# 1dayac/spades_for_blackbird

Hardware: AMD Instinct MI355X
Metric: distinct k-mers/sec (k=21, 150 bp synthetic reads, count only) (higher is better)
Workload: dtype u64

## Files before the change

### spades_for_blackbird_amd/csrc/msd.hip

```cpp
#include <hip/hip_runtime.h>

#include <algorithm>
#include <chrono>
#include <cmath>
#include <cstdio>
#include <cstdlib>
#include <cstring>
#include <optional>
#include <type_traits>
#include <vector>

#include "bbk_internal.h"
#include "kmer_ops.h"
#include "msd.h"

namespace bbk {

#ifndef BBK_KEYS_TILE
#define BBK_KEYS_TILE 8192
#endif
#ifndef BBK_KEYS_THREADS
#define BBK_KEYS_THREADS 512
#endif
template <int W>
// ... 2620 lines not shown
    uint32_t vals[kItems] = {};
    part_tail<1, kItems, kThreads, MAXB, false, false>(keys, vals, binrank, lhist, lstart, goff, scan_tmp, stage,
                                                       vals_unused, nb, T.gbin0, L, cursor, out, nullptr, 0, 0ull);
}

static size_t part_view_smem() {
    return part_smem(1, PartCfg<1>::TILE, false, false, true) + (size_t)kViewSpan * (4 + 2);
}

__global__ void k_view_recanon(const uint64_t *__restrict__ in, const uint32_t *__restrict__ seg_off,
                               const uint32_t *__restrict__ seg_size, int k, uint64_t *__restrict__ out, uint64_t cap,
                               uint32_t *__restrict__ count) {
    const uint32_t o = seg_off[blockIdx.x], n = seg_size[blockIdx.x];
    const uint64_t mask = (1ull << (2 * k)) - 1ull;
    const int lane = threadIdx.x & 63;
    for (uint32_t i0 = 0; i0 < n; i0 += blockDim.x) {
        const uint32_t i = i0 + threadIdx.x;
        Key<1> x;
        x.w[0] = 0;
        bool keep = false;
        if (i < n) {
            x.w[0] = in[o + i] & mask;
            keep = !kmer_less_nucl<1>(kmer_rc<1>(x, k), x);
        }
        const uint64_t bal = __ballot(keep);
        uint32_t base = 0;
        if (lane == 0 && bal) base = atomicAdd(count, (uint32_t)__popcll(bal));
        base = __shfl(base, 0);
        const uint64_t at = (uint64_t)base + __popcll(bal & ((1ull << lane) - 1ull));
        if (keep && at < cap) out[at] = x.w[0];
    }
}

void BucketView::materialise(bbk_ctx *ctx) {
    if (!live()) return;
    keys.alloc(n() * 8 + 16);
    if (nbuckets) {
        KernelTimer t(ctx, "compact", (double)D * (4 + 8));
        hipLaunchKernelGGL(k_compact_narrow<false>, dim3((unsigned)(((uint64_t)nbuckets * 64 + 255) / 256)), dim3(256), 0,
                           ctx->stream, slots.as<uint32_t>(), nullptr, dcount.as<uint32_t>(), off.as<uint64_t>(), nbuckets,
                           stride, seg.as<uint16_t>(), hb, keys.as<uint64_t>(), nullptr);
        check_launch("compact");
    }
    if (n_extra)
        BBK_HIP(bbk::copy_async(keys.as<uint64_t>() + D, extra.p, n_extra * 8, hipMemcpyDeviceToDevice, ctx->stream));
    stream_wait(ctx);
    release_slots();
}

template <int W>
struct BktCfg {
#ifndef BBK_BKT_NT
#define BBK_BKT_NT 512
#define BBK_BKT_ITEMS 11
#endif
#ifndef BBK_BKT2_NT
#define BBK_BKT2_NT 512
#define BBK_BKT2_ITEMS 7
#endif
    static constexpr int NT = (W == 1) ? BBK_BKT_NT : BBK_BKT2_NT;
    static constexpr int ITEMS = (W == 1) ? BBK_BKT_ITEMS : (W == 2 ? BBK_BKT2_ITEMS : (W == 3 ? 5 : 3));
    static constexpr uint32_t CAP = NT * ITEMS;
    static constexpr int NT2 = 512;
    static constexpr int ITEMS2 = (W == 1) ? 23 : (W == 2 ? 11 : (W == 3 ? 7 : 5));
    static constexpr uint32_t CAP2 = NT2 * ITEMS2;
};
constexpr double kBucketFill = 0.70;

static double wall() { return std::chrono::duration<double>(std::chrono::steady_clock::now().time_since_epoch()).count(); }

struct MsdKnobs {
    struct PerProcess {
        bool no_dist = getenv("BBK_NO_DIST") != nullptr;
        uint32_t hash_max_probes = (uint32_t)env_u64(getenv("BBK_HASH_MAX_PROBES"), kHashMaxProbes);
        uint64_t pass_limit = env_u64(getenv("BBK_PASS_LIMIT"), 0);
        bool no_narrow = getenv("BBK_NO_NARROW") != nullptr;
        bool xcd_slots = env_u64(getenv("BBK_XCD_SLOTS"), 1) != 0;
        bool xcd_tiles = env_u64(getenv("BBK_XCD_TILES"), 1) != 0;
        bool no_narrow_b = getenv("BBK_NO_NARROW_B") != nullptr;
        bool no_bucket_handoff = getenv("BBK_NO_BUCKET_HANDOFF") != nullptr;
        uint32_t nw_wgs_per_cu = (uint32_t)env_u64(getenv("BBK_NW_WGS_PER_CU"), 0);
    };
    const PerProcess &once = *[] {
        static const PerProcess p;
        return &p;
    }();
    bool no_slots = getenv("BBK_NO_SLOTS") != nullptr;
    bool no_kslots = getenv("BBK_NO_KSLOTS") != nullptr;
    uint64_t slots_min = env_u64(getenv("BBK_SLOTS_MIN"), 1ull << 22);
    bool verbose = getenv("BBK_VERBOSE") != nullptr;
    bool no_direct = getenv("BBK_NO_DIRECT") != nullptr;
    bool no_level0 = getenv("BBK_NO_LEVEL0") != nullptr;
    bool no_part_kslots = getenv("BBK_NO_PART_KSLOTS") != nullptr;
};

enum class Outcome {
    Declined,
    Done,
    TooBig,
    SlotsGaveUp,
    KeySlotsGaveUp,
    NeedDense,
};

struct MsdInput {
    const bbk_reads *rd;
    const void *keys;
    const uint32_t *vals;
    uint64_t n;
    bool with_mask;
    BucketView *view = nullptr;
};
// ... 96 lines not shown
    }

    double plan_fill(bool from_reads) const { return (!from_reads && use_hash_dedup()) ? 0.52 : kBucketFill; }
    uint64_t pass_limit(bool from_reads) const {
        if (knobs.once.pass_limit) return knobs.once.pass_limit;
        return (uint64_t)(plan_fill(from_reads) * 512 * 0.75 * kMaxBins * bucket_cap() * 0.98);
    }

    struct Sel {
        uint32_t lo = 0, span = 0;
        int shl = 0;
        uint32_t mul = 0;
        uint64_t est = 0;
        void finish() {
            shl = __builtin_clz(span - 1u);
            const uint64_t S = (uint64_t)span << shl;
            mul = S >= (1ull << 32) ? 0u : (uint32_t)((((1ull << 32) - S) << 32) / S);
        }
    };
    struct Dst {
        void *keys = nullptr;
        uint32_t *vals = nullptr;
    };

    struct Plan {
        uint64_t N;
        uint64_t Ntot;
        double target;
        uint32_t nb1 = 1;
        int b1 = 0;
        bool too_deep;
        int nw_hb;
        bool narrow, hslots, kslots, slots;
        uint32_t rd_tile, ntiles1, ntiles1h;
        int xs;
        uint32_t nsub, sub_cap, seg_cap, cap2, stride2, spill_cap;
        size_t rec_ab;
    };

    Plan plan(uint64_t N, uint64_t n_chunks, bool from_reads, bool has_val, const Sel &sel, bool has_dst) const {
        Plan P;
        const bool ranged = sel.span != 0;
        P.Ntot = N;
        P.N = N = ranged ? sel.est : N;
        BBK_REQUIRE(N < (1ull << 32) - kPartTileK, BBK_ERR_ARG,
                    "batch holds %llu records%s; one pass is limited to 2^32-1 (split the input)",
                    (unsigned long long)N, ranged ? " in one range of the prefix space" : "");

        const double fill = plan_fill(from_reads);
        P.target = fill * bucket_cap();
        const double want = std::max(1.0, std::ceil((double)N / P.target));
        while (P.nb1 < 512 && (double)P.nb1 * P.nb1 < want) {
            P.nb1 <<= 1;
            ++P.b1;
        }
        const int ref_bits = dmode == MSD_REF ? std::max(0, 4 - (ranged ? sel.shl : 0)) : 0;
        if (P.b1 < ref_bits) {
            P.b1 = ref_bits;
            P.nb1 = 1u << P.b1;
        }
        const bool u32_slots = (double)N / fill * 1.1 + (double)N < 4.2e9;
        P.nw_hb = (int)(2 * k) - 32;
        P.narrow = W == 1 && from_reads && !ranged && !has_dst && P.nw_hb >= 1 && P.nw_hb <= 10 && slots_ok &&
                   dmode == MSD_HASH && use_hash_dedup() && N >= knobs.slots_min && !knobs.once.no_narrow && u32_slots &&
                   (double)N / kNwBins1 / P.target < 0.75 * kMaxBins;
        if (P.narrow) {
            P.b1 = 10;
            P.nb1 = kNwBins1;
        }
        P.too_deep = want / P.nb1 > 0.75 * kMaxBins;
        if (P.too_deep) return P;

        P.rd_tile = P.narrow ? (uint32_t)(has_val ? NwCfg<true>::CHUNKS : NwCfg<false>::CHUNKS) : (uint32_t)kRdThreads;
        P.ntiles1 = from_reads ? (uint32_t)((n_chunks + P.rd_tile - 1) / P.rd_tile)
                               : (uint32_t)((P.Ntot + kPartTileK - 1) / kPartTileK);
        P.ntiles1h = (uint32_t)((n_chunks + kRdHistThreads - 1) / kRdHistThreads);

        P.hslots = slots_ok && !has_dst && dmode == MSD_HASH && (use_hash_dedup() || use_hashidx_dedup()) && P.nb1 > 1 &&
                   N >= knobs.slots_min && u32_slots;
        P.kslots = kslots_ok && slots_ok && (even_part || (!has_dst && !ranged && expand_k != 0)) && !from_reads &&
                   assume_distinct && (dmode == MSD_KEYS || dmode == MSD_REF) && P.nb1 > 1 && N >= knobs.slots_min &&
                   !knobs.no_direct && u32_slots;
        P.slots = P.hslots || P.kslots;
        BBK_REQUIRE(!P.narrow || P.slots, BBK_ERR_INTERNAL, "narrow records need the slot mode");
        P.xs = (P.slots && knobs.once.xcd_slots && ctx->num_xcds == 8) ? 3 : 0;
        P.nsub = P.nb1 << P.xs;
        P.sub_cap = P.xs ? ((uint32_t)((double)N / P.nsub * 1.06) + 2048u) | 1u : 0u;
        P.seg_cap = !P.slots ? 0u
                    : P.xs   ? P.sub_cap << P.xs
                             : ((uint32_t)((double)N / P.nb1 * (P.kslots ? 1.06 : 1.01)) + 8192u) | 1u;
        P.cap2 = P.narrow ? (uint32_t)(kNwHashThreads * kNwHashItems) : bucket_cap();
        P.rec_ab = P.narrow ? 4 : rec;
        P.stride2 = P.cap2 + (uint32_t)(256 / P.rec_ab);
        P.spill_cap = P.slots ? (uint32_t)(N / 8 + 65536) : 0u;
        return P;
    }

    struct Pass {
        static constexpr uint32_t kFlagCap = 65536;
        MsdRunner &R;
        bbk_ctx *ctx;
        const MsdInput &in;
        MsdOutput &out;
        const Sel sel;
        const Dst dst;
        const bool from_reads, has_val, ranged, has_dst, out_vals, need_vbuf, verbose;
        Plan P{};
        uint64_t N = 0, n_chunks = 0;
        DevBuf coff, tile_read, tiles_h;
        enum { kCtlSpill = 0, kCtlUnordered = 4, kCtlDup = 8, kCtlFlagN = 12, kCtlDbg = 16, kCtlTotal = 32, kCtlWords = 40 };
        DevBuf ctl;
        uint32_t h_ctl[kCtlWords] = {};
        uint32_t *ctl_at(int w) const { return ctl.as<uint32_t>() + w; }
        uint64_t *ctl_total() const { return reinterpret_cast<uint64_t *>(ctl_at(kCtlTotal)); }
        uint64_t h_total() const {
            uint64_t t;
            memcpy(&t, h_ctl + kCtlTotal, 8);
            return t;
        }
        ReadSrc S{}, Sh{};
        TileMap M1{}, M2{};
        PartLevel L1{}, L2{};
        DevBuf spill_k, spill_v;
        DevBuf hist1, cur1, bufA, valA;
        uint32_t n32 = 0;
        std::vector<uint32_t> h1, off1, tstart, snb2, sbin, hsub, fill1;
        std::vector<uint32_t> over_seg;
        uint32_t nbuckets = 0, ntiles2 = 0, nwg2 = 0;
        bool narrow_b = false;
        uint32_t *stage = nullptr;
        DevBuf layout_d;
        uint32_t *seg_tile = nullptr, *seg_off = nullptr, *seg_nb2 = nullptr, *seg_bin = nullptr, *seg_size = nullptr,
                 *xstart_d = nullptr;
        DevBuf desc2, desc2h, hist2, boff, bufB, valB;
        std::vector<uint32_t> xstart;
        DevBuf dcount, slot_off, bseg, bbase, flag_ids;
        DevBuf c64, d64;
        bool d64_scanned = false;
        std::vector<DevBuf> scan_keep;
        BucketArgs A{};
        bool direct = false;
        uint32_t ctr[4] = {0, 0, 0, 0};
        std::vector<uint32_t> flagged, hd, hb;
        std::vector<uint32_t> big;
        uint32_t hbo[2] = {0, 0};
        MsdOutput extra;
        uint64_t novf = 0;

        Pass(MsdRunner &r, const MsdInput &i, MsdOutput &o, const Sel &s, Dst d)
            : R(r), ctx(r.ctx), in(i), out(o), sel(s), dst(d), from_reads(i.rd != nullptr),
              has_val(i.with_mask || i.vals != nullptr), ranged(s.span != 0), has_dst(d.keys != nullptr),
              out_vals(r.op != MSD_OP_NONE), need_vbuf(has_val || out_vals), verbose(r.knobs.verbose) {}

        double rec_bytes(uint64_t n) const { return (double)n * (rec + (has_val ? 4 : 0)); }
        uint32_t *vals_or_null(DevBuf &b) const { return has_val ? b.as<uint32_t>() : nullptr; }

        Outcome run(uint64_t *n_records = nullptr) {
            ctl.alloc(kCtlWords * 4);
            BBK_HIP(hipMemsetAsync(ctl.p, 0, kCtlWords * 4, ctx->stream));
            count_instances();
            out.instances = N;
            out.n = 0;
            if (N == 0) return empty();
            if (!ranged && n_records && N > R.pass_limit(from_reads)) {
                *n_records = N;
                return Outcome::TooBig;
            }
            P = R.plan(N, n_chunks, from_reads, has_val, sel, has_dst);
            N = P.N;
            if (in.view && !view_level1()) return Outcome::NeedDense;
            if (P.too_deep) {
                if (verbose) fprintf(stderr, "[bbk] msd declines: N=%llu needs more than two levels\n", (unsigned long long)N);
                return Outcome::Declined;
            }
            level1_tiles();
            if (auto r = level1()) return *r;
            level2_layout();
            level2_scatter();
            if (auto r = first_pass()) return *r;
            if (auto r = overflow()) return *r;
            compact();
            return Outcome::Done;
        }

        bool view_level1() const {
            return W == 1 && !P.too_deep && P.kslots && R.expand_k && !ranged && !has_dst && !R.even_part && !has_val;
        }

        Outcome empty() {
            if (!has_dst) {
                out.keys.alloc(16);
                out.vals.alloc(16);
            }
            return Outcome::Done;
        }

        void count_instances() {
            N = (R.expand_k && !from_reads) ? 2 * in.n : in.n;
            if (!from_reads) return;
            const bbk_reads *rd = in.rd;
            BBK_REQUIRE(R.dmode == MSD_HASH, BBK_ERR_INTERNAL, "reads are partitioned by hash prefix only");
// ... 103 lines not shown
            if (P.narrow) {
                if constexpr (W == 1) {
                    const double pbn = (double)in.rd->n_words * 8 + (double)N * (4 + (has_val ? 4 : 0));
                    const uint32_t per_cu = R.knobs.once.nw_wgs_per_cu;
                    const uint32_t grid = per_cu ? std::min<uint32_t>(P.ntiles1, (uint32_t)ctx->num_cus * per_cu) : P.ntiles1;
                    R.launch(has_val ? k_part_reads_narrow<true> : k_part_reads_narrow<false>, "k_part_reads_narrow", pbn,
                             grid, kNwThreads, part_reads_narrow_smem(has_val), S, L1, P.ntiles1, S.tiles,
                             cur1.as<uint32_t>(), bufA.as<uint32_t>(), vals_or_null(valA));
                }
            } else {
                const double pb = (from_reads ? (double)in.rd->n_words * 8 : rec_bytes(N)) + rec_bytes(N);
                if (from_reads)
                    R.template launch_part_reads<false>("k_part_reads", pb, P.ntiles1, has_val, S, L1, nullptr,
                                                        cur1.as<uint32_t>(), bufA.as<Key<W>>(), valA.as<uint32_t>());
                else if (in.view)
                    level1_from_view();
                else
                    R.template scatter_keys<true>(has_val, "k_part_l1", pb, P.ntiles1, (const Key<W> *)in.keys, in.vals, M1, L1,
                                   cur1.as<uint32_t>(), bufA.as<Key<W>>(), valA.as<uint32_t>());
            }
            if (!P.slots) return std::nullopt;
            auto r = slot_fills();
            if (in.view && !r) {
                in.view->release_slots();
                if (verbose) fprintf(stderr, "[bbk] msd key slots: level 1 read stage A's buckets (%llu + %llu keys)\n",
                                     (unsigned long long)in.view->D, (unsigned long long)in.view->n_extra);
            }
            return r;
        }

        void level1_from_view() {
            if constexpr (W == 1) {
                BucketView &v = *in.view;
                const uint32_t half = kPartTileK / 2;
                const uint32_t nt = (uint32_t)((v.D + half - 1) / half);
                if (nt) {
                    DevBuf vdesc((size_t)nt * sizeof(uint2) + 16);
                    hipLaunchKernelGGL(k_view_tile_desc, dim3((nt + 255) / 256), dim3(256), 0, ctx->stream,
                                       v.off.as<uint64_t>(), v.nbuckets, v.D, half, nt, vdesc.as<uint2>());
                    check_launch("k_view_tile_desc");
                    TileMap Mv = M1;
                    Mv.n = 2 * v.D;
                    Mv.ntiles = nt;
                    R.launch(R.expand_tag ? k_part_view<true> : k_part_view<false>, "k_part_view",
                             (double)v.D * 4 + 2.0 * (double)v.D * rec, nt, PartCfg<1>::THREADS, part_view_smem(),
                             v.slots.as<uint32_t>(), v.off.as<uint64_t>(), v.seg.as<uint16_t>(), vdesc.as<uint2>(),
                             v.stride, v.hb, Mv, L1, cur1.as<uint32_t>(), bufA.as<Key<1>>());
                }
                if (v.n_extra) {
                    TileMap Me = M1;
                    Me.n = 2 * v.n_extra;
                    const uint32_t nte = (uint32_t)((Me.n + kPartTileK - 1) / kPartTileK);
                    R.template scatter_keys<true>(false, "k_part_l1", rec_bytes(v.n_extra) + rec_bytes(Me.n), nte,
                                                  v.extra.as<Key<W>>(), nullptr, Me, L1, cur1.as<uint32_t>(),
                                                  bufA.as<Key<W>>(), nullptr);
                }
            }
        }

        Outcome give_up_key_slots() {
            if constexpr (W == 1) {
                if (in.view && !in.view->live() && !in.view->keys.p) {
                    BucketView &v = *in.view;
                    const uint64_t n = v.n();
                    v.keys.alloc(n * rec + 16);
                    DevBuf cnt(16);
                    BBK_HIP(hipMemsetAsync(cnt.p, 0, 16, ctx->stream));
                    hipLaunchKernelGGL(k_view_recanon, dim3(P.nsub), dim3(256), 0, ctx->stream, bufA.as<uint64_t>(),
                                       seg_off, seg_size, (int)R.expand_k,
                                       v.keys.as<uint64_t>(), n, cnt.as<uint32_t>());
                    check_launch("k_view_recanon");
                    uint32_t got = 0;
                    BBK_HIP(hipMemcpyAsync(&got, cnt.p, 4, hipMemcpyDeviceToHost, ctx->stream));
                    stream_wait(ctx);
                    BBK_REQUIRE(got == n, BBK_ERR_INTERNAL, "canonical keys rebuilt from level 1: %u of %llu", got,
                                (unsigned long long)n);
                }
            }
            return Outcome::KeySlotsGaveUp;
        }

        std::optional<Outcome> slot_fills() {
            const uint32_t nsub = P.nsub, xs = P.xs;
            std::vector<uint32_t> c1(nsub);
            BBK_HIP(hipMemcpyAsync(c1.data(), cur1.p, (size_t)nsub * 4, hipMemcpyDeviceToHost, ctx->stream));
            stream_wait(ctx);
            uint64_t got = 0;
            const uint32_t cap1 = xs ? P.sub_cap : P.seg_cap;
            for (uint32_t b = 0; b < P.nb1; ++b) {
                bool over = false;
                uint32_t tot = 0;
                for (uint32_t s2 = b << xs; s2 < (b + 1) << xs; ++s2) {
                    const uint32_t reserved = c1[s2] - off1[s2];
                    got += reserved;
                    over = over || reserved > cap1;
                    fill1[s2] = std::min(reserved, cap1);
                    tot += fill1[s2];
                }
                if (over) over_seg.push_back(b);
                h1[b] = over ? 0u : tot;
                for (uint32_t s2 = b << xs; s2 < (b + 1) << xs; ++s2) hsub[s2] = over ? 0u : fill1[s2];
            }
            if (got > P.Ntot) {
// ... 13 lines not shown
                            (unsigned long long)got, (unsigned long long)P.Ntot);
            }
            if (ranged) {
                N = got;
                out.instances = N;
            }
            BBK_REQUIRE(got == N, BBK_ERR_INTERNAL, "level-1 reservations do not add up (%llu vs %llu)",
                        (unsigned long long)got, (unsigned long long)N);
            if (N == 0) return empty();
            if (P.kslots && !over_seg.empty()) {
                if (verbose) fprintf(stderr, "[bbk] msd key slots: %zu segments overflow, exact mode\n", over_seg.size());
                return Outcome::KeySlotsGaveUp;
            }
            return std::nullopt;
        }

        static size_t pad4(size_t words) { return (words + 7) & ~(size_t)3; }
        size_t layout_words(uint32_t *off_w) const {
            const size_t len[6] = {(size_t)P.nsub + 1, (size_t)P.nsub + 1, P.nb1, (size_t)P.nb1 + 1, P.nsub, P.nsub};
            size_t at = 0;
            for (int i = 0; i < 6; ++i) {
                if (off_w) off_w[i] = (uint32_t)at;
                at += pad4(len[i]);
            }
            return at;
        }

        void level2_layout() {
            const uint32_t nb1 = P.nb1, nsub = P.nsub, xs = P.xs;
            if (!P.slots)
                for (uint32_t b = 0; b < nb1; ++b) hsub[b] = h1[b];
            tstart[0] = 0;
            sbin[0] = 0;
            const uint32_t tile2 = P.narrow ? (uint32_t)(has_val ? Nw2Cfg<true>::TILE : Nw2Cfg<false>::TILE) : kPartTileK;
            for (uint32_t s2 = 0; s2 < nsub; ++s2) tstart[s2 + 1] = tstart[s2] + (hsub[s2] + tile2 - 1) / tile2;
            for (uint32_t b = 0; b < nb1; ++b) {
                snb2[b] = (uint32_t)std::min<double>(kMaxBins, std::max(1.0, std::ceil((double)h1[b] / P.target)));
                sbin[b + 1] = sbin[b] + snb2[b];
            }
            nbuckets = sbin[nb1];

            const int w0bits = R.w0bits();
            uint64_t span_b = 0;
            for (uint32_t b = 0; b < nb1; ++b)
                if (h1[b]) {
                    const uint64_t Q = 1ull << (32 - P.b1), q = (Q + snb2[b] - 1) / snb2[b];
                    span_b = std::max(span_b, w0bits > 32 ? q << (w0bits - 32) : q >> (32 - w0bits));
                }
            narrow_b = W == 1 && P.kslots && !R.even_part && !ranged && !has_dst && !has_val && R.op == MSD_OP_NONE &&
                       R.dmode == MSD_KEYS && span_b <= (1ull << 32) && !R.knobs.once.no_narrow_b;
            if (P.kslots && verbose)
                fprintf(stderr, "[bbk] msd key slots: %s records from level 2 (widest bucket 2^%.1f keys)\n",
                        narrow_b ? "4-byte" : "8-byte", std::log2((double)std::max<uint64_t>(span_b, 1)));

            ntiles2 = tstart[nsub];
            nwg2 = ntiles2;
            if (R.knobs.once.xcd_tiles && ntiles2) {
                xstart.resize(nsub);
                uint32_t per_xcd[8] = {0, 0, 0, 0, 0, 0, 0, 0};
                for (uint32_t s2 = 0; s2 < nsub; ++s2) {
                    uint32_t &c = per_xcd[(s2 >> xs) & 7u];
                    xstart[s2] = c;
                    c += tstart[s2 + 1] - tstart[s2];
                }
                nwg2 = 8u * *std::max_element(per_xcd, per_xcd + 8);
            }
            uint32_t off_w[6];
            const size_t words = layout_words(off_w);
            layout_d.alloc(words * 4);
            uint32_t *h = stage + pad4(nsub), *d = layout_d.as<uint32_t>();
            memcpy(h + off_w[0], tstart.data(), ((size_t)nsub + 1) * 4);
            memcpy(h + off_w[1], off1.data(), ((size_t)nsub + 1) * 4);
            memcpy(h + off_w[2], snb2.data(), (size_t)nb1 * 4);
            memcpy(h + off_w[3], sbin.data(), ((size_t)nb1 + 1) * 4);
            memcpy(h + off_w[4], hsub.data(), (size_t)nsub * 4);
            if (!xstart.empty()) memcpy(h + off_w[5], xstart.data(), (size_t)nsub * 4);
            BBK_HIP(hipMemcpyAsync(d, h, words * 4, hipMemcpyHostToDevice, ctx->stream));
            seg_tile = d + off_w[0];
            seg_off = d + off_w[1];
            seg_nb2 = d + off_w[2];
            seg_bin = d + off_w[3];
            seg_size = d + off_w[4];
            xstart_d = xstart.empty() ? nullptr : d + off_w[5];
            L2 = PartLevel{2, P.b1, nb1, R.dmode, w0bits, seg_nb2, seg_bin, sel.lo, sel.span, sel.shl, sel.mul};
            M2 = TileMap{seg_tile, seg_off, seg_size, nsub, N, ntiles2, 1, nullptr, 0, 0};
            desc2.alloc((size_t)nwg2 * sizeof(uint4) + 16);
            if (ntiles2) {
                if (xstart_d) BBK_HIP(hipMemsetAsync(desc2.p, 0, (size_t)nwg2 * sizeof(uint4), ctx->stream));
                hipLaunchKernelGGL(P.narrow ? k_tile_desc_narrow : k_tile_desc, dim3((ntiles2 + 255) / 256), dim3(256), 0,
                                   ctx->stream, M2, seg_nb2, seg_bin, tile2, xs, (const uint32_t *)xstart_d,
                                   desc2.as<uint4>());
                check_launch("k_tile_desc");
            }
            M2.desc = desc2.as<uint4>();
            if (!P.slots && xstart_d && !P.narrow) {
                desc2h.alloc((size_t)ntiles2 * sizeof(uint4) + 16);
                hipLaunchKernelGGL(k_tile_desc, dim3((ntiles2 + 255) / 256), dim3(256), 0, ctx->stream, M2, seg_nb2, seg_bin,
                                   kPartTileK, xs, (const uint32_t *)nullptr, desc2h.as<uint4>());
                check_launch("k_tile_desc");
            }
        }

        void level2_scatter() {
            hist2.alloc((size_t)nbuckets * 4 + 16);
            boff.alloc(((size_t)nbuckets + 1) * 4 + 16);
            const uint64_t nB = P.slots ? (uint64_t)nbuckets * P.stride2 : N;
            if (P.slots) BBK_REQUIRE(nB + N < (1ull << 32), BBK_ERR_INTERNAL, "slot layout exceeds 32-bit offsets");
            bufB.alloc(nB * (narrow_b ? 4 : P.rec_ab));
            if (need_vbuf) valB.alloc(nB * 4);
            if (!P.slots) {
                BBK_HIP(hipMemsetAsync(hist2.p, 0, (size_t)nbuckets * 4 + 16, ctx->stream));
                TileMap M2h = M2;
                if (desc2h.p) M2h.desc = desc2h.as<uint4>();
                R.template launch_part<false, true, false>("k_part_hist2", (double)N * rec, ntiles2, bufA.as<Key<W>>(), nullptr,
                                                    M2h, L2, hist2.as<uint32_t>(), nullptr, nullptr, nullptr);
                DevBuf h64(((size_t)nbuckets + 1) * 8);
                hipLaunchKernelGGL(k_u32_to_u64, dim3((nbuckets + 255) / 256), dim3(256), 0, ctx->stream,
                                   hist2.as<uint32_t>(), (uint64_t)nbuckets, h64.as<uint64_t>(), 0u);
                check_launch("k_u32_to_u64");
                const uint64_t tot = exclusive_scan_u64(ctx, h64.as<uint64_t>(), h64.as<uint64_t>(), nbuckets);
                BBK_REQUIRE(tot == N, BBK_ERR_INTERNAL, "level-2 histogram does not add up");
                hipLaunchKernelGGL(k_scan_to_u32, dim3((nbuckets + 1 + 255) / 256), dim3(256), 0, ctx->stream,
                                   h64.as<uint64_t>(), (uint64_t)nbuckets, tot, (const uint64_t *)nullptr,
                                   boff.as<uint32_t>());
                check_launch("k_scan_to_u32");
                BBK_HIP(bbk::copy_async(hist2.p, boff.p, (size_t)nbuckets * 4, hipMemcpyDeviceToDevice, ctx->stream));
                stream_wait(ctx);
            } else {
                if (P.narrow) bseg.alloc(((size_t)nbuckets + 1) * 2);
                hipLaunchKernelGGL(k_bucket_init, dim3((nbuckets + 255) / 256), dim3(256), 0, ctx->stream,
                                   hist2.as<uint32_t>(), nbuckets, P.stride2, (const uint32_t *)seg_bin, P.nb1,
                                   P.narrow ? bseg.as<uint16_t>() : (uint16_t *)nullptr);
                check_launch("k_bucket_init");
                use_slots(L2, P.cap2, P.stride2);
            }
            if (P.narrow) {
                if (ntiles2)
                    R.launch(has_val ? k_part_narrow2<true> : k_part_narrow2<false>, "k_part_narrow2",
                             2.0 * (double)N * (4 + (has_val ? 4 : 0)), nwg2, kNw2Threads, part_narrow2_smem(has_val),
                             bufA.as<uint32_t>(), vals_or_null(valA), desc2.as<uint4>(), L2, hist2.as<uint32_t>(),
                             bufB.as<uint32_t>(), vals_or_null(valB));
            } else if (narrow_b) {
                if constexpr (W == 1)
                    R.template launch_part<false, false, false, true>("k_part_l2", (double)N * (rec + 4), nwg2,
                                                                        bufA.as<Key<W>>(), nullptr, M2, L2, nullptr,
                                                                        hist2.as<uint32_t>(), bufB.as<Key<W>>(), nullptr);
            } else {
                R.template scatter_keys<false>(has_val, "k_part_l2", 2.0 * rec_bytes(N), nwg2, bufA.as<Key<W>>(), valA.as<uint32_t>(), M2,
                               L2, hist2.as<uint32_t>(), bufB.as<Key<W>>(), valB.as<uint32_t>());
            }
        }

        std::optional<Outcome> first_pass() {
            dcount.alloc((size_t)nbuckets * 4 + 16);
            A = BucketArgs{boff.as<uint32_t>(), dcount.as<uint32_t>(), nullptr, (int)R.k,
                           verbose ? ctl_at(kCtlDbg) : nullptr, P.slots ? P.cap2 : 0u, P.slots ? P.stride2 : 0u,
                           hist2.as<uint32_t>(), nullptr, nullptr, nullptr, ~0ull, R.knobs.once.hash_max_probes, nullptr};
            direct = (!P.slots || P.kslots) && R.assume_distinct && (R.dmode == MSD_KEYS || R.dmode == MSD_REF) &&
                     !R.knobs.no_direct;
            if (P.kslots) {
                c64.alloc(((size_t)nbuckets + 1) * 8);
                const ScanSrc src{hist2.p, SCAN_SLOT_FILL, P.stride2, P.cap2};
                uint64_t *const so = c64.as<uint64_t>();
                exclusive_scan_enqueue(ctx, 1, &src, &so, nbuckets, ctl_total(), false, scan_keep);
                slot_off.alloc(((size_t)nbuckets + 1) * 4 + 16);
                hipLaunchKernelGGL(k_scan_to_u32, dim3((nbuckets + 1 + 255) / 256), dim3(256), 0, ctx->stream,
                                   c64.as<uint64_t>(), (uint64_t)nbuckets, 0ull, (const uint64_t *)ctl_total(),
                                   slot_off.as<uint32_t>());
                check_launch("k_scan_to_u32");
                A.out_off = slot_off.as<uint32_t>();
            }
            if (direct) {
                if (!has_dst) {
                    out.keys.alloc(N * rec + 16);
                    if (out_vals) out.vals.alloc(N * 4 + 16);
                }
                A.sorted_keys = has_dst ? dst.keys : out.keys.p;
                A.sorted_vals = has_dst ? dst.vals : out.vals.as<uint32_t>();
                A.dup_flag = ctl_at(kCtlDup);
                A.strip_mask = R.strip_mask;
            }
            launch_buckets();
            flag_ids.alloc((size_t)kFlagCap * 4);
            if (P.hslots && !direct) {
                d64.alloc(((size_t)nbuckets + 1) * 8);
                const ScanSrc src{dcount.p, SCAN_U32_FLAGGED, 0u, 0u};
                uint64_t *const so = d64.as<uint64_t>();
                exclusive_scan_enqueue(ctx, 1, &src, &so, nbuckets, ctl_total(), false, scan_keep);
                d64_scanned = true;
            }
            fetch_flags();
            if (P.kslots && h_total() != N) {
                if (verbose) fprintf(stderr, "[bbk] msd key slots: %llu of %llu records placed, exact mode\n",
                                     (unsigned long long)h_total(), (unsigned long long)N);
                out.keys.release();
                out.vals.release();
                return give_up_key_slots();
            }
            if (!direct) return std::nullopt;
            if (ctr[2] == 0 && ctr[3] == 0 && (!P.kslots || ctr[0] == 0)) {
                out.n = N;
                out.nbuckets = 0;
// ... 8 lines not shown
                                     ctr[2], ctr[3]);
                out.keys.release();
                out.vals.release();
                return give_up_key_slots();
            }
            if (verbose) fprintf(stderr, "[bbk] msd direct output withdrawn (flagged=%u dup=%u): in-place pass\n", ctr[2], ctr[3]);
            if (!has_dst) {
                out.keys.release();
                out.vals.release();
            }
            A.sorted_keys = nullptr;
            A.sorted_vals = nullptr;
            A.dup_flag = nullptr;
            A.strip_mask = ~0ull;
            R.template bucket_dispatch<false>(nbuckets, bufB.as<Key<W>>(), valB.as<uint32_t>(), A, rec_bytes(N));
            fetch_flags();
            return std::nullopt;
        }

        void launch_buckets() {
            if (P.narrow) {
                if constexpr (W == 1) {
                    if (nbuckets)
                        with_op(R.op, [&](auto o) {
                            constexpr int OP = decltype(o)::value;
                            R.launch(k_bucket_hash32<OP>, "k_bucket_hash32", (double)N * (4 + (has_val ? 4 : 0)), nbuckets,
                                     kNwHashThreads, bucket_hash32_smem<OP>(), bufB.as<uint32_t>(), valB.as<uint32_t>(), A,
                                     bseg.as<uint16_t>(), P.nw_hb);
                        });
                }
            } else if (narrow_b) {
                if constexpr (W == 1) {
                    BBK_REQUIRE(direct, BBK_ERR_INTERNAL, "4-byte stage-B records need the direct output");
                    bbase.alloc(((size_t)nbuckets + 1) * 8);
                    if (nbuckets) {
                        hipLaunchKernelGGL(k_bucket_base, dim3((nbuckets + 255) / 256), dim3(256), 0, ctx->stream,
                                           (const uint32_t *)seg_nb2, (const uint32_t *)seg_bin, P.nb1, nbuckets, P.b1,
                                           R.w0bits(), bbase.as<uint64_t>());
                        check_launch("k_bucket_base");
                        constexpr int NT = BktCfg<1>::NT, IT = BktCfg<1>::ITEMS;
                        R.launch(k_bucket_dist_nb<NT, IT>, "k_bucket_dist", (double)N * (4 + rec), nbuckets, NT,
                                 bucket_dist_nb_smem<NT, IT>(), bufB.as<uint32_t>(), bbase.as<uint64_t>(), A);
                    }
                }
            } else {
                R.template bucket_dispatch<false>(nbuckets, bufB.as<Key<W>>(), valB.as<uint32_t>(), A, rec_bytes(N));
            }
        }

        void fetch_flags() {
            uint32_t *d_flag_n = P.slots ? ctl_at(kCtlSpill) + 2 : ctl_at(kCtlFlagN);
            if (!P.slots) BBK_HIP(hipMemsetAsync(d_flag_n, 0, 16, ctx->stream));
            hipLaunchKernelGGL(k_flagged, dim3((nbuckets + 255) / 256), dim3(256), 0, ctx->stream, dcount.as<uint32_t>(),
                               nbuckets, flag_ids.as<uint32_t>(), kFlagCap, d_flag_n);
            check_launch("k_flagged");
            BBK_HIP(hipMemcpyAsync(h_ctl, ctl.p, kCtlWords * 4, hipMemcpyDeviceToHost, ctx->stream));
            stream_wait(ctx);
            if (P.slots) memcpy(ctr, h_ctl + kCtlSpill, 12);
            else ctr[2] = h_ctl[kCtlFlagN];
            if (direct) ctr[3] = h_ctl[kCtlDup];
        }

        std::optional<Outcome> overflow() {
            const uint32_t n_flag = ctr[2];
            if (n_flag > kFlagCap) {
                if (verbose) fprintf(stderr, "[bbk] msd: %u buckets overflow\n", n_flag);
                return P.slots ? Outcome::SlotsGaveUp : Outcome::Declined;
            }
            flagged.resize(n_flag);
            if (n_flag) {
                BBK_HIP(hipMemcpyAsync(flagged.data(), flag_ids.p, (size_t)n_flag * 4, hipMemcpyDeviceToHost, ctx->stream));
                stream_wait(ctx);
// ... 642 lines not shown
```

Baseline: 27.90 billion.

## Use 4-byte records from level 1 with hash tag applied at level 2

Adds a 'late tag' path for key-slot partitioning from a view. Level 1 now emits 4-byte low-bit records binned by the top 10 bits of both orientations, and the hash tag is computed only at level 2. Level 2 then folds the tag into its bin index, and new permutation kernels reorder the slot-fill scan to match. The goal is to halve record traffic in the first partition pass. The cost is a more complex bucket mapping, extra small kernels, and a forced 1024-bin level 1.

```diff
diff --git a/spades_for_blackbird_amd/csrc/msd.hip b/spades_for_blackbird_amd/csrc/msd.hip
--- a/spades_for_blackbird_amd/csrc/msd.hip
+++ b/spades_for_blackbird_amd/csrc/msd.hip
@@ -2676,6 +2676,321 @@
     }
 }
 
+constexpr int kLtThreads = 1024;
+constexpr int kLt1Items = 14;
+constexpr int kLt2Items = 12;
+
+struct LtLds {
+    uint32_t *lhist;
+    uint2 *tab;
+    uint32_t *lstart, *scan_tmp;
+    unsigned long long *mark;
+    uint16_t *mbase, *nz;
+    uint32_t *stage;
+};
+template <int ITEMS>
+__device__ __forceinline__ LtLds lt_lds(unsigned char *smem) {
+    constexpr int MW = kLtThreads * ITEMS / 64;
+    LtLds S;
+    S.lhist = reinterpret_cast<uint32_t *>(smem);
+    S.tab = reinterpret_cast<uint2 *>(smem);
+    S.lstart = S.lhist + 2 * kMaxBins;
+    S.scan_tmp = S.lstart + kMaxBins;
+    S.mark = reinterpret_cast<unsigned long long *>(S.scan_tmp + 64);
+    S.mbase = reinterpret_cast<uint16_t *>(S.mark + MW);
+    S.nz = S.mbase + MW;
+    S.stage = reinterpret_cast<uint32_t *>(S.nz + kMaxBins);
+    return S;
+}
+static size_t lt_smem(int items, size_t more) {
+    const size_t tile = (size_t)kLtThreads * items;
+    return sizeof(uint32_t) * (3 * kMaxBins + 64) + (tile / 64) * (8 + 2) + (size_t)kMaxBins * 2 + tile * 4 + more;
+}
+
+__device__ inline uint64_t lt_tagged(uint32_t seg, uint32_t lo, int lobits, int k) {
+    Key<1> x;
+    x.w[0] = ((uint64_t)seg << lobits) | lo;
+    return x.w[0] | (__umul64hi(xxh3_64<1>(x), 16ull) << (2 * k));
+}
+
+template <int ITEMS, class KeyOf>
+__device__ __forceinline__ void lt_tail(const LtLds &S, const uint32_t (&lo)[ITEMS], const uint32_t (&bins)[ITEMS / 2],
+                                        uint32_t nb, uint32_t *__restrict__ cur, uint64_t slot_end, uint32_t rec_or,
+                                        const PartLevel &L, uint32_t *__restrict__ out, KeyOf key_of) {
+    constexpr int NT = kLtThreads, MW = NT * ITEMS / 64;
+    static_assert(ITEMS % 2 == 0 && ITEMS <= 32 && NT * ITEMS < 65536, "packed bins, one bit per item, 16-bit positions");
+    const uint32_t tid = threadIdx.x;
+    const int lane = tid & 63, wave = tid >> 6;
+    const uint32_t c = tid < nb ? S.lhist[tid] : 0u;
+    uint32_t incl = c;
+    incl = wave_scan_incl(incl);
+    const unsigned long long nzb = __ballot(c != 0);
+    if (lane == 63) S.scan_tmp[wave] = incl | ((uint32_t)__popcll(nzb) << 16);
+    __syncthreads();
+    uint32_t before, total;
+    wave_totals<NT / 64>(S.scan_tmp, lane, wave, before, total);
+    const uint32_t staged = total & 0xFFFFu;
+    const uint32_t ex = (before & 0xFFFFu) + incl - c;
+    const uint32_t myr = (before >> 16) + (uint32_t)__popcll(nzb & ((1ull << lane) - 1ull));
+    S.lstart[tid] = ex;
+    uint32_t greserve = 0;
+    if (c) {
+        greserve = atomicAdd(cur, c);
+        S.nz[myr] = (uint16_t)tid;
+        atomicOr(&S.mark[ex >> 6], 1ull << (ex & 63u));
+    }
+    __syncthreads();
+#pragma unroll
+    for (int i = 0; i < ITEMS; ++i) {
+        const uint32_t bin = (bins[i >> 1] >> (16 * (i & 1))) & 0xFFFFu;
+        if (bin != 0xFFFFu) {
+            const uint32_t pos = atomicAdd(&S.lstart[bin], 1u);
+            S.stage[pos] = lo[i];
+        }
+    }
+    asm volatile("" : "+v"(greserve));
+    if (c) {
+        const int64_t room = (int64_t)slot_end - (int64_t)greserve;
+        S.tab[myr] = make_uint2(greserve - ex, (uint32_t)(int32_t)(room < -(int64_t)0x7FFF0000 ? -(int64_t)0x7FFF0000 : room) + ex);
+    }
+    if (wave == 0) {
+        constexpr int WPL = (MW + 63) / 64;
+        uint32_t pw[WPL], tot = 0;
+#pragma unroll
+        for (int j = 0; j < WPL; ++j) {
+            const int idx = lane * WPL + j;
+            pw[j] = tot;
+            tot += idx < MW ? (uint32_t)__popcll(S.mark[idx]) : 0u;
+        }
+        uint32_t inc2 = tot;
+        inc2 = wave_scan_incl(inc2);
+        const uint32_t lb = inc2 - tot;
+#pragma unroll
+        for (int j = 0; j < WPL; ++j) {
+            const int idx = lane * WPL + j;
+            if (idx < MW) S.mbase[idx] = (uint16_t)(lb + pw[j]);
+        }
+    }
+    __syncthreads();
+    const unsigned long long upto = (2ull << lane) - 1ull;
+    const unsigned long long *wmark = S.mark + wave;
+    const uint16_t *wmbase = S.mbase + wave;
+    uint32_t full = 0;
+#pragma unroll
+    for (int i = 0; i < ITEMS; ++i) {
+        const uint32_t pos = (uint32_t)i * NT + tid;
+        if (pos < staged) {
+            const uint32_t r = (uint32_t)wmbase[i * (NT / 64)] + (uint32_t)__popcll(wmark[i * (NT / 64)] & upto) - 1u;
+            unsigned long long e = reinterpret_cast<const unsigned long long *>(S.tab)[r];
+            const uint32_t rec = S.stage[pos];
+            asm volatile("" : "+v"(e));
+            if ((int32_t)pos >= (int32_t)(uint32_t)(e >> 32)) full |= 1u << i;
+            else out[(uint32_t)e + pos] = rec | rec_or;
+        }
+    }
+    if (full) {
+#pragma unroll 1
+        for (int i = 0; i < ITEMS; ++i) {
+            if ((full >> i) & 1u) {
+                const uint32_t pos = (uint32_t)i * NT + tid;
+                const uint32_t r = (uint32_t)wmbase[i * (NT / 64)] + (uint32_t)__popcll(wmark[i * (NT / 64)] & upto) - 1u;
+                const uint32_t sp = atomicAdd(L.spill_count, 1u);
+                if (sp < L.spill_cap) reinterpret_cast<uint64_t *>(L.spill_keys)[sp] = key_of((uint32_t)S.nz[r], S.stage[pos]);
+            }
+        }
+    }
+}
+
+template <bool DENSE>
+__global__ __launch_bounds__(kLtThreads) __attribute__((amdgpu_waves_per_eu(8, 8))) void k_part_view_lt(
+    const uint32_t *__restrict__ slots, const uint64_t *__restrict__ off, const uint16_t *__restrict__ seg,
+    const uint2 *__restrict__ vdesc, uint32_t stride, int hb, const uint64_t *__restrict__ dense, uint64_t nkeys_all, int k,
+    PartLevel L, uint32_t *__restrict__ cursor, uint32_t *__restrict__ out) {
+    constexpr int NT = kLtThreads, ITEMS = kLt1Items, KPT = NT * ITEMS / 2, MW = NT * ITEMS / 64;
+    extern __shared__ __attribute__((aligned(16))) unsigned char smem[];
+    const LtLds S = lt_lds<ITEMS>(smem);
+    uint32_t *toff = S.stage + NT * ITEMS;
+    uint16_t *tseg = reinterpret_cast<uint16_t *>(toff + kViewSpan);
+    const uint32_t tid = threadIdx.x;
+    uint32_t xcc = 0;
+    if (L.xcd_shift) {
+        asm volatile("s_getreg_b32 %0, hwreg(HW_REG_XCC_ID)" : "=s"(xcc));
+        xcc &= (1u << L.xcd_shift) - 1u;
+    }
+    const int lobits = 2 * k - 10;
+    const uint32_t lomask = lobits >= 32 ? 0xFFFFFFFFu : (1u << lobits) - 1u;
+    const uint64_t c0 = (uint64_t)blockIdx.x * KPT;
+    const uint64_t left = nkeys_all - c0;
+    const uint32_t nkeys = left < (uint64_t)KPT ? (uint32_t)left : (uint32_t)KPT;
+    uint32_t b0 = 0, span = 0;
+    bool staged_tab = false;
+    if (!DENSE) {
+        const uint2 d = vdesc[blockIdx.x];
+        b0 = d.x;
+        span = d.y - d.x + 1u;
+        staged_tab = span <= (uint32_t)kViewSpan;
+        if (staged_tab && tid < span) {
+            toff[tid] = (uint32_t)off[b0 + tid];
+            tseg[tid] = seg[b0 + tid];
+        }
+    }
+    S.lhist[tid] = 0;
+    if (tid < 2 * MW) reinterpret_cast<uint32_t *>(S.mark)[tid] = 0u;
+    __syncthreads();
+
+    uint64_t x[ITEMS / 2];
+    if (DENSE) {
+#pragma unroll
+        for (int j = 0; j < ITEMS / 2; ++j) {
+            const uint32_t cl = (uint32_t)(j * NT) + tid;
+            x[j] = dense[c0 + (cl < nkeys ? cl : nkeys - 1u)];
+        }
+    } else {
+        uint32_t w[ITEMS / 2], sg[ITEMS / 2];
+#pragma unroll
+        for (int j = 0; j < ITEMS / 2; ++j) {
+            const uint32_t cl = (uint32_t)(j * NT) + tid;
+            const uint32_t c = (uint32_t)c0 + (cl < nkeys ? cl : nkeys - 1u);
+            uint32_t b, base;
+            if (staged_tab) {
+                uint32_t i = 0, hi = span;
+                while (hi - i > 1) {
+                    const uint32_t mid = (i + hi) >> 1;
+                    if (toff[mid] <= c) i = mid;
+                    else hi = mid;
+                }
+                b = b0 + i;
+                base = toff[i];
+                sg[j] = tseg[i];
+            } else {
+                b = view_bucket(off, b0, b0 + span, c);
+                base = (uint32_t)off[b];
+                sg[j] = seg[b];
+            }
+            w[j] = slots[(size_t)b * stride + (c - base)];
+        }
+#pragma unroll
+        for (int j = 0; j < ITEMS / 2; ++j) x[j] = nw_key(sg[j], w[j], hb);
+    }
+    uint32_t lo[ITEMS], bins[ITEMS / 2];
+#pragma unroll
+    for (int j = 0; j < ITEMS / 2; ++j) {
+        Key<1> a;
+        a.w[0] = x[j];
+        const uint64_t r = kmer_rc<1>(a, k).w[0];
+        const uint32_t ba = (uint32_t)(x[j] >> lobits), br = (uint32_t)(r >> lobits);
+        lo[2 * j] = (uint32_t)x[j] & lomask;
+        lo[2 * j + 1] = (uint32_t)r & lomask;
+        bins[j] = 0xFFFFFFFFu;
+        if ((uint32_t)(j * NT) + tid < nkeys) {
+            bins[j] = ba | (br << 16);
+            atomicAdd(&S.lhist[ba], 1u);
+            atomicAdd(&S.lhist[br], 1u);
+        }
+    }
+    __syncthreads();
+    const uint64_t slot_end = (uint64_t)tid * L.slot_stride + (L.xcd_shift ? (uint64_t)(xcc + 1u) * L.sub_cap : (uint64_t)L.slot_cap);
+    lt_tail<ITEMS>(S, lo, bins, (uint32_t)kMaxBins, &cursor[(tid << L.xcd_shift) + xcc], slot_end, 0u, L, out,
+                   [&](uint32_t bin, uint32_t rec) { return lt_tagged(bin, rec, lobits, k); });
+}
+
+__global__ __launch_bounds__(kLtThreads) __attribute__((amdgpu_waves_per_eu(8, 8))) void k_part_lt2(
+    const uint32_t *__restrict__ in, const uint4 *__restrict__ desc, int k, PartLevel L, uint32_t *__restrict__ cursor,
+    uint32_t *__restrict__ out) {
+    constexpr int NT = kLtThreads, ITEMS = kLt2Items, MW = NT * ITEMS / 64;
+    extern __shared__ __attribute__((aligned(16))) unsigned char smem[];
+    const LtLds S = lt_lds<ITEMS>(smem);
+    const uint32_t tid = threadIdx.x;
+    const uint4 d = desc[blockIdx.x];
+    const uint32_t begin = d.x, count = d.y, nb = d.z & 0xFFFFu, sgm = d.z >> 16, gbin0 = d.w;
+    if (count == 0) return;
+    const int lobits = 2 * k - 10;
+    const uint32_t nsub = nb >> 4;
+    const uint64_t segbits = (uint64_t)sgm << lobits;
+    S.lhist[tid] = 0;
+    if (tid < 2 * MW) reinterpret_cast<uint32_t *>(S.mark)[tid] = 0u;
+    __syncthreads();
+    uint32_t lo[ITEMS], bins[ITEMS / 2];
+#pragma unroll
+    for (int i = 0; i < ITEMS; ++i) {
+        const uint32_t local = (uint32_t)i * NT + tid;
+        lo[i] = in[begin + (local < count ? local : count - 1u)];
+    }
+#pragma unroll
+    for (int i = 0; i < ITEMS; ++i) asm volatile("" : "+v"(lo[i]));
+#pragma unroll
+    for (int i = 0; i < ITEMS; ++i) {
+        Key<1> x;
+        x.w[0] = segbits | lo[i];
+        const uint32_t tag = (uint32_t)__umul64hi(xxh3_64<1>(x), 16ull);
+        const uint32_t b = tag * nsub + __umulhi(lo[i] << (32 - lobits), nsub);
+        const bool valid = (uint32_t)i * NT + tid < count;
+        if (valid) atomicAdd(&S.lhist[b], 1u);
+        const uint32_t b16 = valid ? b : 0xFFFFu;
+        if (i & 1) bins[i >> 1] |= b16 << 16;
+        else bins[i >> 1] = b16;
+    }
+    __syncthreads();
+    const uint64_t slot_end = (uint64_t)(gbin0 + tid) * L.slot_stride + L.slot_cap;
+    lt_tail<ITEMS>(S, lo, bins, nb, &cursor[gbin0 + tid], slot_end, (uint32_t)segbits, L, out,
+                   [&](uint32_t, uint32_t rec) { return lt_tagged(sgm, rec, lobits, k); });
+}
+
+__global__ void k_bucket_base_lt(const uint32_t *__restrict__ seg_nb2, const uint32_t *__restrict__ seg_bin, uint32_t nseg,
+                                 uint32_t nbuckets, int lobits, int k, uint64_t *__restrict__ base,
+                                 uint32_t *__restrict__ perm) {
+    const uint32_t g = blockIdx.x * blockDim.x + threadIdx.x;
+    if (g >= nbuckets) return;
+    uint32_t lo = 0, hi = nseg;
+    while (hi - lo > 1) {
+        const uint32_t mid = (lo + hi) >> 1;
+        if (seg_bin[mid] <= g) lo = mid;
+        else hi = mid;
+    }
+    const uint32_t nsub = seg_nb2[lo] >> 4, r = g - seg_bin[lo], tag = r / nsub, j = r - tag * nsub;
+    const uint64_t q = (((uint64_t)j << lobits) + nsub - 1u) / nsub;
+    base[g] = ((uint64_t)tag << (2 * k)) | ((uint64_t)lo << lobits) | q;
+    perm[g] = tag * (nbuckets >> 4) + (seg_bin[lo] >> 4) + j;
+}
+
+__global__ void k_lt_fill_perm(const uint32_t *__restrict__ cursor, const uint32_t *__restrict__ perm, uint32_t n,
+                               uint32_t stride, uint32_t cap, uint32_t *__restrict__ fill) {
+    const uint32_t g = blockIdx.x * blockDim.x + threadIdx.x;
+    if (g >= n) return;
+    const uint32_t c = cursor[g] - g * stride;
+    fill[perm[g]] = c < cap ? c : cap;
+}
+
+__global__ void k_lt_unperm(const uint64_t *__restrict__ scanned, const uint32_t *__restrict__ perm, uint32_t n,
+                            uint32_t *__restrict__ out_off) {
+    const uint32_t g = blockIdx.x * blockDim.x + threadIdx.x;
+    if (g < n) out_off[g] = (uint32_t)scanned[perm[g]];
+}
+
+__global__ void k_view_recanon_lt(const uint32_t *__restrict__ in, const uint32_t *__restrict__ seg_off,
+                                  const uint32_t *__restrict__ seg_size, int sub_shift, int k, uint64_t *__restrict__ out,
+                                  uint64_t cap, uint32_t *__restrict__ count) {
+    const uint32_t o = seg_off[blockIdx.x], n = seg_size[blockIdx.x];
+    const uint64_t segbits = (uint64_t)(blockIdx.x >> sub_shift) << (2 * k - 10);
+    const int lane = threadIdx.x & 63;
+    for (uint32_t i0 = 0; i0 < n; i0 += blockDim.x) {
+        const uint32_t i = i0 + threadIdx.x;
+        Key<1> x;
+        x.w[0] = 0;
+        bool keep = false;
+        if (i < n) {
+            x.w[0] = segbits | in[o + i];
+            keep = !kmer_less_nucl<1>(kmer_rc<1>(x, k), x);
+        }
+        const uint64_t bal = __ballot(keep);
+        uint32_t base = 0;
+        if (lane == 0 && bal) base = atomicAdd(count, (uint32_t)__popcll(bal));
+        base = __shfl(base, 0);
+        const uint64_t at = (uint64_t)base + __popcll(bal & ((1ull << lane) - 1ull));
+        if (keep && at < cap) out[at] = x.w[0];
+    }
+}
+
 void BucketView::materialise(bbk_ctx *ctx) {
     if (!live()) return;
     keys.alloc(n() * 8 + 16);
@@ -2722,6 +3037,7 @@
         bool xcd_slots = env_u64(getenv("BBK_XCD_SLOTS"), 1) != 0;
         bool xcd_tiles = env_u64(getenv("BBK_XCD_TILES"), 1) != 0;
         bool no_narrow_b = getenv("BBK_NO_NARROW_B") != nullptr;
+        bool no_late_tag = getenv("BBK_NO_LATE_TAG") != nullptr;
         bool no_bucket_handoff = getenv("BBK_NO_BUCKET_HANDOFF") != nullptr;
         uint32_t nw_wgs_per_cu = (uint32_t)env_u64(getenv("BBK_NW_WGS_PER_CU"), 0);
     };
@@ -2884,13 +3200,15 @@
         bool too_deep;
         int nw_hb;
         bool narrow, hslots, kslots, slots;
+        bool late_tag = false;
         uint32_t rd_tile, ntiles1, ntiles1h;
         int xs;
         uint32_t nsub, sub_cap, seg_cap, cap2, stride2, spill_cap;
         size_t rec_ab;
     };
 
-    Plan plan(uint64_t N, uint64_t n_chunks, bool from_reads, bool has_val, const Sel &sel, bool has_dst) const {
+    Plan plan(uint64_t N, uint64_t n_chunks, bool from_reads, bool has_val, const Sel &sel, bool has_dst,
+              bool from_view = false) const {
         Plan P;
         const bool ranged = sel.span != 0;
         P.Ntot = N;
@@ -2935,6 +3253,19 @@
                    !knobs.no_direct && u32_slots;
         P.slots = P.hslots || P.kslots;
         BBK_REQUIRE(!P.narrow || P.slots, BBK_ERR_INTERNAL, "narrow records need the slot mode");
+        P.late_tag = false;
+        if (W == 1 && from_view && P.kslots && expand_tag && !even_part && !ranged && !has_dst && !has_val &&
+            op == MSD_OP_NONE && dmode == MSD_KEYS && !knobs.once.no_narrow_b && !knobs.once.no_late_tag && expand_k >= 17 &&
+            2 * expand_k <= 42) {
+            const double nb2 = std::min<double>(kMaxBins, std::max(1.0, std::ceil((double)N / P.nb1 / P.target)));
+            const uint64_t Q = 1ull << (32 - P.b1), q = (Q + (uint64_t)nb2 - 1) / (uint64_t)nb2;
+            const int wb = w0bits();
+            P.late_tag = (wb > 32 ? q << (wb - 32) : q >> (32 - wb)) <= (1ull << 32);
+        }
+        if (P.late_tag) {
+            P.b1 = 10;
+            P.nb1 = kMaxBins;
+        }
         P.xs = (P.slots && knobs.once.xcd_slots && ctx->num_xcds == 8) ? 3 : 0;
         P.nsub = P.nb1 << P.xs;
         P.sub_cap = P.xs ? ((uint32_t)((double)N / P.nsub * 1.06) + 2048u) | 1u : 0u;
@@ -2942,7 +3273,7 @@
                     : P.xs   ? P.sub_cap << P.xs
                              : ((uint32_t)((double)N / P.nb1 * (P.kslots ? 1.06 : 1.01)) + 8192u) | 1u;
         P.cap2 = P.narrow ? (uint32_t)(kNwHashThreads * kNwHashItems) : bucket_cap();
-        P.rec_ab = P.narrow ? 4 : rec;
+        P.rec_ab = (P.narrow || P.late_tag) ? 4 : rec;
         P.stride2 = P.cap2 + (uint32_t)(256 / P.rec_ab);
         P.spill_cap = P.slots ? (uint32_t)(N / 8 + 65536) : 0u;
         return P;
@@ -2987,6 +3318,7 @@
         DevBuf desc2, desc2h, hist2, boff, bufB, valB;
         std::vector<uint32_t> xstart;
         DevBuf dcount, slot_off, bseg, bbase, flag_ids;
+        DevBuf bperm, pfill;
         DevBuf c64, d64;
         bool d64_scanned = false;
         std::vector<DevBuf> scan_keep;
@@ -3018,7 +3350,7 @@
                 *n_records = N;
                 return Outcome::TooBig;
             }
-            P = R.plan(N, n_chunks, from_reads, has_val, sel, has_dst);
+            P = R.plan(N, n_chunks, from_reads, has_val, sel, has_dst, in.view != nullptr);
             N = P.N;
             if (in.view && !view_level1()) return Outcome::NeedDense;
             if (P.too_deep) {
@@ -3188,6 +3520,10 @@
         void level1_from_view() {
             if constexpr (W == 1) {
                 BucketView &v = *in.view;
+                if (P.late_tag) {
+                    level1_late_tag(v);
+                    return;
+                }
                 const uint32_t half = kPartTileK / 2;
                 const uint32_t nt = (uint32_t)((v.D + half - 1) / half);
                 if (nt) {
@@ -3214,6 +3550,32 @@
             }
         }
 
+        void level1_late_tag(BucketView &v) {
+            if constexpr (W == 1) {
+                constexpr uint32_t kpt = (uint32_t)kLtThreads * kLt1Items / 2;
+                const size_t lds = lt_smem(kLt1Items, (size_t)kViewSpan * (4 + 2));
+                const uint32_t nt = (uint32_t)((v.D + kpt - 1) / kpt);
+                ctx->add_stat("stat_late_tag", (double)N);
+                if (nt) {
+                    DevBuf vdesc((size_t)nt * sizeof(uint2) + 16);
+                    hipLaunchKernelGGL(k_view_tile_desc, dim3((nt + 255) / 256), dim3(256), 0, ctx->stream,
+                                       v.off.as<uint64_t>(), v.nbuckets, v.D, kpt, nt, vdesc.as<uint2>());
+                    check_launch("k_view_tile_desc");
+                    R.launch(k_part_view_lt<false>, "k_part_view", (double)v.D * 4 + 2.0 * (double)v.D * 4, nt, kLtThreads, lds,
+                             v.slots.as<uint32_t>(), v.off.as<uint64_t>(), v.seg.as<uint16_t>(), vdesc.as<uint2>(), v.stride,
+                             v.hb, (const uint64_t *)nullptr, v.D, (int)R.expand_k, L1, cur1.as<uint32_t>(),
+                             bufA.as<uint32_t>());
+                }
+                if (v.n_extra) {
+                    const uint32_t nte = (uint32_t)((v.n_extra + kpt - 1) / kpt);
+                    R.launch(k_part_view_lt<true>, "k_part_l1", (double)v.n_extra * 8 + 2.0 * (double)v.n_extra * 4, nte,
+                             kLtThreads, lds, (const uint32_t *)nullptr, (const uint64_t *)nullptr, (const uint16_t *)nullptr,
+                             (const uint2 *)nullptr, 0u, 0, v.extra.as<uint64_t>(), v.n_extra, (int)R.expand_k, L1,
+                             cur1.as<uint32_t>(), bufA.as<uint32_t>());
+                }
+            }
+        }
+
         Outcome give_up_key_slots() {
             if constexpr (W == 1) {
                 if (in.view && !in.view->live() && !in.view->keys.p) {
@@ -3222,9 +3584,16 @@
                     v.keys.alloc(n * rec + 16);
                     DevBuf cnt(16);
                     BBK_HIP(hipMemsetAsync(cnt.p, 0, 16, ctx->stream));
-                    hipLaunchKernelGGL(k_view_recanon, dim3(P.nsub), dim3(256), 0, ctx->stream, bufA.as<uint64_t>(),
-                                       seg_off, seg_size, (int)R.expand_k,
-                                       v.keys.as<uint64_t>(), n, cnt.as<uint32_t>());
+                    if (P.late_tag) {
+                        ctx->add_stat("stat_late_tag_recanon", (double)n);
+                        hipLaunchKernelGGL(k_view_recanon_lt, dim3(P.nsub), dim3(256), 0, ctx->stream, bufA.as<uint32_t>(),
+                                           seg_off, seg_size, P.xs, (int)R.expand_k, v.keys.as<uint64_t>(), n,
+                                           cnt.as<uint32_t>());
+                    } else {
+                        hipLaunchKernelGGL(k_view_recanon, dim3(P.nsub), dim3(256), 0, ctx->stream, bufA.as<uint64_t>(),
+                                           seg_off, seg_size, (int)R.expand_k, v.keys.as<uint64_t>(), n,
+                                           cnt.as<uint32_t>());
+                    }
                     check_launch("k_view_recanon");
                     uint32_t got = 0;
                     BBK_HIP(hipMemcpyAsync(&got, cnt.p, 4, hipMemcpyDeviceToHost, ctx->stream));
@@ -3304,10 +3673,13 @@
                 for (uint32_t b = 0; b < nb1; ++b) hsub[b] = h1[b];
             tstart[0] = 0;
             sbin[0] = 0;
-            const uint32_t tile2 = P.narrow ? (uint32_t)(has_val ? Nw2Cfg<true>::TILE : Nw2Cfg<false>::TILE) : kPartTileK;
+            const uint32_t tile2 = P.late_tag ? (uint32_t)(kLtThreads * kLt2Items)
+                                   : P.narrow   ? (uint32_t)(has_val ? Nw2Cfg<true>::TILE : Nw2Cfg<false>::TILE)
+                                                : kPartTileK;
             for (uint32_t s2 = 0; s2 < nsub; ++s2) tstart[s2 + 1] = tstart[s2] + (hsub[s2] + tile2 - 1) / tile2;
             for (uint32_t b = 0; b < nb1; ++b) {
-                snb2[b] = (uint32_t)std::min<double>(kMaxBins, std::max(1.0, std::ceil((double)h1[b] / P.target)));
+                snb2[b] = P.late_tag ? 16u * (uint32_t)std::min<double>(kMaxBins / 16, std::max(1.0, std::ceil((double)h1[b] / (16.0 * P.target))))
+                                     : (uint32_t)std::min<double>(kMaxBins, std::max(1.0, std::ceil((double)h1[b] / P.target)));
                 sbin[b + 1] = sbin[b] + snb2[b];
             }
             nbuckets = sbin[nb1];
@@ -3321,7 +3693,10 @@
                 }
             narrow_b = W == 1 && P.kslots && !R.even_part && !ranged && !has_dst && !has_val && R.op == MSD_OP_NONE &&
                        R.dmode == MSD_KEYS && span_b <= (1ull << 32) && !R.knobs.once.no_narrow_b;
-            if (P.kslots && verbose)
+            if (P.late_tag) narrow_b = true;
+            if (P.late_tag && verbose)
+                fprintf(stderr, "[bbk] msd key slots: 4-byte records from level 1, tag taken at level 2 (%u buckets)\n", nbuckets);
+            else if (P.kslots && verbose)
                 fprintf(stderr, "[bbk] msd key slots: %s records from level 2 (widest bucket 2^%.1f keys)\n",
                         narrow_b ? "4-byte" : "8-byte", std::log2((double)std::max<uint64_t>(span_b, 1)));
 
@@ -3359,7 +3734,7 @@
             desc2.alloc((size_t)nwg2 * sizeof(uint4) + 16);
             if (ntiles2) {
                 if (xstart_d) BBK_HIP(hipMemsetAsync(desc2.p, 0, (size_t)nwg2 * sizeof(uint4), ctx->stream));
-                hipLaunchKernelGGL(P.narrow ? k_tile_desc_narrow : k_tile_desc, dim3((ntiles2 + 255) / 256), dim3(256), 0,
+                hipLaunchKernelGGL((P.narrow || P.late_tag) ? k_tile_desc_narrow : k_tile_desc, dim3((ntiles2 + 255) / 256), dim3(256), 0,
                                    ctx->stream, M2, seg_nb2, seg_bin, tile2, xs, (const uint32_t *)xstart_d,
                                    desc2.as<uint4>());
                 check_launch("k_tile_desc");
@@ -3412,6 +3787,12 @@
                              2.0 * (double)N * (4 + (has_val ? 4 : 0)), nwg2, kNw2Threads, part_narrow2_smem(has_val),
                              bufA.as<uint32_t>(), vals_or_null(valA), desc2.as<uint4>(), L2, hist2.as<uint32_t>(),
                              bufB.as<uint32_t>(), vals_or_null(valB));
+            } else if (P.late_tag) {
+                if constexpr (W == 1)
+                    if (ntiles2)
+                        R.launch(k_part_lt2, "k_part_l2", 2.0 * (double)N * 4, nwg2, kLtThreads, lt_smem(kLt2Items, 0),
+                                 bufA.as<uint32_t>(), desc2.as<uint4>(), (int)R.expand_k, L2, hist2.as<uint32_t>(),
+                                 bufB.as<uint32_t>());
             } else if (narrow_b) {
                 if constexpr (W == 1)
                     R.template launch_part<false, false, false, true>("k_part_l2", (double)N * (rec + 4), nwg2,
@@ -3432,14 +3813,33 @@
                      !R.knobs.no_direct;
             if (P.kslots) {
                 c64.alloc(((size_t)nbuckets + 1) * 8);
-                const ScanSrc src{hist2.p, SCAN_SLOT_FILL, P.stride2, P.cap2};
                 uint64_t *const so = c64.as<uint64_t>();
-                exclusive_scan_enqueue(ctx, 1, &src, &so, nbuckets, ctl_total(), false, scan_keep);
                 slot_off.alloc(((size_t)nbuckets + 1) * 4 + 16);
-                hipLaunchKernelGGL(k_scan_to_u32, dim3((nbuckets + 1 + 255) / 256), dim3(256), 0, ctx->stream,
-                                   c64.as<uint64_t>(), (uint64_t)nbuckets, 0ull, (const uint64_t *)ctl_total(),
-                                   slot_off.as<uint32_t>());
-                check_launch("k_scan_to_u32");
+                if (P.late_tag) {
+                    const dim3 gb((nbuckets + 255) / 256);
+                    bbase.alloc(((size_t)nbuckets + 1) * 8);
+                    bperm.alloc(((size_t)nbuckets + 1) * 4);
+                    pfill.alloc(((size_t)nbuckets + 1) * 4);
+                    hipLaunchKernelGGL(k_bucket_base_lt, gb, dim3(256), 0, ctx->stream, (const uint32_t *)seg_nb2,
+                                       (const uint32_t *)seg_bin, P.nb1, nbuckets, 2 * (int)R.expand_k - 10, (int)R.expand_k,
+                                       bbase.as<uint64_t>(), bperm.as<uint32_t>());
+                    check_launch("k_bucket_base_lt");
+                    hipLaunchKernelGGL(k_lt_fill_perm, gb, dim3(256), 0, ctx->stream, hist2.as<uint32_t>(),
+                                       bperm.as<uint32_t>(), nbuckets, P.stride2, P.cap2, pfill.as<uint32_t>());
+                    check_launch("k_lt_fill_perm");
+                    const ScanSrc src{pfill.p, SCAN_U32_FLAGGED, 0u, 0u};
+                    exclusive_scan_enqueue(ctx, 1, &src, &so, nbuckets, ctl_total(), false, scan_keep);
+                    hipLaunchKernelGGL(k_lt_unperm, gb, dim3(256), 0, ctx->stream, c64.as<uint64_t>(), bperm.as<uint32_t>(),
+                                       nbuckets, slot_off.as<uint32_t>());
+                    check_launch("k_lt_unperm");
+                } else {
+                    const ScanSrc src{hist2.p, SCAN_SLOT_FILL, P.stride2, P.cap2};
+                    exclusive_scan_enqueue(ctx, 1, &src, &so, nbuckets, ctl_total(), false, scan_keep);
+                    hipLaunchKernelGGL(k_scan_to_u32, dim3((nbuckets + 1 + 255) / 256), dim3(256), 0, ctx->stream,
+                                       c64.as<uint64_t>(), (uint64_t)nbuckets, 0ull, (const uint64_t *)ctl_total(),
+                                       slot_off.as<uint32_t>());
+                    check_launch("k_scan_to_u32");
+                }
                 A.out_off = slot_off.as<uint32_t>();
             }
             if (direct) {
@@ -3514,12 +3914,14 @@
             } else if (narrow_b) {
                 if constexpr (W == 1) {
                     BBK_REQUIRE(direct, BBK_ERR_INTERNAL, "4-byte stage-B records need the direct output");
-                    bbase.alloc(((size_t)nbuckets + 1) * 8);
+                    if (!P.late_tag) bbase.alloc(((size_t)nbuckets + 1) * 8);
                     if (nbuckets) {
-                        hipLaunchKernelGGL(k_bucket_base, dim3((nbuckets + 255) / 256), dim3(256), 0, ctx->stream,
-                                           (const uint32_t *)seg_nb2, (const uint32_t *)seg_bin, P.nb1, nbuckets, P.b1,
-                                           R.w0bits(), bbase.as<uint64_t>());
-                        check_launch("k_bucket_base");
+                        if (!P.late_tag) {
+                            hipLaunchKernelGGL(k_bucket_base, dim3((nbuckets + 255) / 256), dim3(256), 0, ctx->stream,
+                                               (const uint32_t *)seg_nb2, (const uint32_t *)seg_bin, P.nb1, nbuckets, P.b1,
+                                               R.w0bits(), bbase.as<uint64_t>());
+                            check_launch("k_bucket_base");
+                        }
                         constexpr int NT = BktCfg<1>::NT, IT = BktCfg<1>::ITEMS;
                         R.launch(k_bucket_dist_nb<NT, IT>, "k_bucket_dist", (double)N * (4 + rec), nbuckets, NT,
                                  bucket_dist_nb_smem<NT, IT>(), bufB.as<uint32_t>(), bbase.as<uint64_t>(), A);
```

Result: faster. 30.23 billion, median of 6 (+8.3%).
